# ai4co/rl4co

Hardware: NVIDIA H100
Metric: node-selections/sec TSP-100 AM rollout (higher is better)
Workload: dtype f32

## Files before the change

### include/corollout.h

```cpp
#ifndef COROLLOUT_H_
#define COROLLOUT_H_

#include <stdint.h>

#ifdef __cplusplus
extern "C" {
#endif

#define CO_VERSION 100

#define CO_OK 0
#define CO_ERR_BAD_ARG (-1)
#define CO_ERR_UNSUPPORTED (-2)
#define CO_ERR_CUDA (-3)

#define CO_EMBED_DIM 128
#define CO_NUM_HEADS 8

#define CO_ENV_TSP 0
#define CO_ENV_CVRP 1
#define CO_ENV_SDVRP 2
#define CO_ENV_OP 3
#define CO_ENV_PCTSP 4

#define CO_SELECT_GREEDY 0
#define CO_SELECT_SAMPLE_NOISE 1
#define CO_SELECT_EVALUATE 2
#define CO_SELECT_SAMPLE_PHILOX 3

int co_version(void);
const char* co_last_error_string(void);
int co_device_sm_count(void);


int co_tsp_step(const int64_t* action, const uint8_t* mask_in, uint8_t* mask_out,
                int64_t* first_node, int64_t* current_node, int64_t* i, uint8_t* done,
                int B, int N, void* stream);

int co_cvrp_action_mask(const float* demand, const float* used_capacity,
                        const float* vehicle_capacity, const uint8_t* visited,
                        const int64_t* current_node, uint8_t* mask_out, int B, int N,
                        void* stream);

int co_cvrp_step(const int64_t* action, const float* demand, const float* vehicle_capacity,
                 const float* used_in, float* used_out, const uint8_t* visited_in,
                 uint8_t* visited_out, int64_t* current_node, uint8_t* done,
                 uint8_t* mask_out, int B, int N, void* stream);

int co_sdvrp_action_mask(const float* demand_with_depot, const float* used_capacity,
                         const float* vehicle_capacity, const int64_t* current_node, uint8_t* mask_out,
                         int B, int N, void* stream);
int co_sdvrp_step(const int64_t* action, const float* demand_in, float* demand_out,
                  const float* vehicle_capacity, const float* used_in, float* used_out,
                  int64_t* current_node, uint8_t* done, uint8_t* mask_out, int B, int N, void* stream);

int co_op_action_mask(const float* locs, const float* max_length, const uint8_t* visited, const float* tour_length,
                      const int64_t* current_node, uint8_t* mask_out, int B, int N, void* stream);
int co_op_step(const int64_t* action, const float* locs, const float* prize, const float* max_length,
               const uint8_t* visited_in, uint8_t* visited_out, float* tour_length, float* current_total_prize,
               int64_t* current_node, int64_t* i, uint8_t* done, uint8_t* mask_out, int B, int N, void* stream);
int co_op_reward(const float* prize, const int64_t* actions, float* reward, int B, int N, int T, void* stream);

int co_pctsp_action_mask(const uint8_t* visited, const float* cur_total_prize, uint8_t* mask_out, int B, int N, void* stream);
int co_pctsp_step(const int64_t* action, const float* real_prize, const float* penalty, const uint8_t* visited_in,
                  uint8_t* visited_out, float* cur_total_prize, float* cur_total_penalty, int64_t* current_node, int64_t* i,
                  uint8_t* done, uint8_t* mask_out, int B, int N, void* stream);

int co_tour_length(const float* locs, const int64_t* actions, float* reward, int B,
                   int B_locs, int N, int T, int with_depot, void* stream);

int co_check_tours(const int64_t* actions, const float* demand,
                   const float* vehicle_capacity, int32_t* bad_count, int B, int B_inst,
                   int N, int T, void* stream);

#define CO_TWO_OPT_MAX_NODES 1024
#define CO_TWO_OPT_RESIDENT_MAX_NODES 224
int co_tsp_two_opt(const float* locs, const float* dist, const int64_t* tours_in, int64_t* tours_out,
                   int32_t* iterations, int B, int N, int max_iterations, void* stream);

int co_cvrp_local_search(const float* locs, const float* dist, const float* demand, const float* capacity,
                         const int64_t* tours_in, int64_t* tours_out, int32_t* used_len, int32_t* iterations,
                         int32_t* feasible, int B, int N, int T, int max_iterations, void* stream);


typedef struct co_decoder_weights {
  const float* project_context_t;
  const float* w_placeholder;
  const float* project_out_t;
  const float* dynamic_w;
  const float* dynamic_feature;
} co_decoder_weights;

int co_pointer_logits(int env_kind, const co_decoder_weights* w, const float* node_emb,
                      const float* graph_ctx ,
                      const float* glimpse_key, const float* glimpse_val,
                      const float* logit_key, const uint8_t* action_mask,
                      const int64_t* first_node, const int64_t* current_node,
                      const int64_t* i, const float* used_capacity,
                      const float* vehicle_capacity, float* logits_out, int B_traj,
                      int B_inst, int N, int ld, void* stream);

int co_select_action(const float* logits, const uint8_t* action_mask, const float* noise,
                     int64_t* action_io, float* logp_out, float* logprobs_out, int mode,
                     float tanh_clipping, float temperature, int mask_logits,
                     uint64_t seed, uint64_t offset, int B, int N, void* stream);


#define CO_ROLLOUT_FORCED_START 1
#define CO_ROLLOUT_NO_PREFETCH 2

typedef struct co_rollout_args {
  int32_t env_kind;
  int32_t select_mode;
  int32_t B_inst;
  int32_t num_starts;
  int32_t N;
  int32_t T_max;
  int32_t num_loc;
  int32_t flags;
  float tanh_clipping;
  float temperature;
  const float* cache;
  const float* graph_ctx;
  const float* q_placeholder;
  const float* w_capacity;
  const float* locs;
  const float* demand;
  const float* vehicle_capacity;
  const int64_t* forced_actions;
  const float* noise;
  uint64_t seed, offset;
  int64_t* actions_out;
  float* logp_out;
  float* reward_out;
  float* loglik_out;
  int32_t* steps_out;
  int32_t* max_steps_out;
  float* used_capacity_out;
  const float* node_emb;
  const float* w_first;
  int32_t cache_width;
  int32_t reserved0;
  const float* dyn_w;
  const float* node_limit;
} co_rollout_args;

typedef struct co_eas_grad_args {
  int32_t env_kind;
  int32_t B_inst;
  int32_t num_rows;
  int32_t N;
  int32_t T;
  int32_t cache_width;
  float tanh_clipping;
  float temperature;
  const float* cache;
  const float* graph_ctx;
  const float* w_capacity;
  const float* demand;
  const float* vehicle_capacity;
  const int64_t* actions;
  const float* coef;
  float* dLf;
  float* loglik;
  int32_t* bad_rows;
} co_eas_grad_args;
int co_eas_key_grad(const co_eas_grad_args* args, void* stream);

int co_cache_width(int env_kind);
int co_rollout_max_nodes(void);
int co_rollout(const co_rollout_args* args, void* stream);

int co_split_tf32(const float* w, float* hi, float* lo, long n, void* stream);
int co_gemm_tf32x3(const float* A, const float* Whi, const float* Wlo, float* C,
                   const float* bias, const float* residual, const float* scale,
                   const float* shift, int M, int Nout, int K, int lda, int ldc, int ldr,
                   int relu, void* stream);

long co_ffn_tiled_weight_floats(void);
int co_ffn_tile_weights(const float* w1hi, const float* w1lo, const float* w2hi, const float* w2lo, float* wtiled,
                        void* stream);
int co_ffn_fused(const float* x, const float* wtiled, const float* b1, const float* b2, const float* scale,
                 const float* shift, float* out, int M, int ldx, int ldo, void* stream);

int co_generate_uniform(float* out, long n, uint64_t seed, uint64_t offset, float lo, float hi, void* stream);
int co_generate_demand(float* out, long n, uint64_t seed, uint64_t offset, int min_demand, int max_demand,
                       float capacity, void* stream);
int co_dihedral8(const float* locs, float* out, long B, int N, void* stream);

int co_symmetric_augment(const float* base, const float* phi, float* out, long B, int S, int N, void* stream);

#define CO_LOCS_MAX_NODES 10000
#define CO_LOCS_UNIFORM 0
#define CO_LOCS_CONSTANT 1
#define CO_LOCS_NORMAL 2
#define CO_LOCS_CLUSTER 3
#define CO_LOCS_MIXED 4
#define CO_LOCS_GAUSSIAN_MIXTURE 5
#define CO_LOCS_MIX_DISTRIBUTION 6
#define CO_LOCS_MIX_MULTI_DISTRIBUTIONS 7
typedef struct co_locs_args {
  int64_t B;
  int32_t N;
  int32_t kind;
  uint64_t seed, offset;
  float lo, hi;
  float mean, std;
  int32_t n_cluster;
  int32_t n_cluster_mix;
  int32_t num_modes;
  float cdist;
} co_locs_args;
int co_generate_locs(float* out, const co_locs_args* args, void* stream);

int co_encoder_mha(const float* qkv, float* out, int B, int N, void* stream);

typedef struct co_attn_args {
  const float* q;
  const float* k;
  const float* v;
  const uint32_t* mask;
  float* o;
  float* lse;
  const float* dO;
  float* dq;
  float* dk;
  float* dv;
  int32_t B, M, N, reserved0;
  int64_t q_bs, k_bs, v_bs, o_bs, dq_bs, dk_bs, dv_bs;
  int32_t q_rs, k_rs, v_rs, o_rs, dq_rs, dk_rs, dv_rs;
  float scale;
} co_attn_args;
int co_attn_fwd(const co_attn_args* args, void* stream);
int co_attn_bwd(const co_attn_args* args, void* stream);

int co_instance_norm(const float* x, const float* gamma, const float* beta, float* out, long B, int N, float eps,
                     void* stream);

int co_reward_stats(const float* reward, double* out2, int B, void* stream);

#ifdef __cplusplus
}
#endif
#endif
```

### rl4co_b200/csrc/gemm_tf32x3.cu

```cuda
#include "co_common.cuh"
#include "wgmma.cuh"

namespace co {

constexpr int GM = 128, GN = 128, GK = 32;
constexpr int TILE_BYTES = GM * GK * 4;
constexpr uint32_t SBO = 1024;
constexpr int KB128 = 4;
constexpr int STAGES = 3;
constexpr int GEMM_THREADS = 384;
constexpr int GEMM_SMEM = 2 * KB128 * TILE_BYTES + STAGES * 2 * TILE_BYTES;

__device__ __forceinline__ float4 split_hi(float4 v) {
  return make_float4(wg::rna_tf32(v.x), wg::rna_tf32(v.y), wg::rna_tf32(v.z), wg::rna_tf32(v.w));
}
__device__ __forceinline__ float4 sub4(float4 a, float4 b) { return make_float4(a.x - b.x, a.y - b.y, a.z - b.z, a.w - b.w); }

__global__ void split_tf32_kernel(const float* __restrict__ w, float* __restrict__ hi, float* __restrict__ lo, long n) {
  long i = (long)blockIdx.x * blockDim.x + threadIdx.x;
  if (i < n) {
    const float v = w[i], h = wg::rna_tf32(v);
    hi[i] = h;
    lo[i] = v - h;
  }
}

struct GemmArgs {
  const float* A; const float* Whi; const float* Wlo; float* C;
  const float* bias; const float* residual; const float* scale; const float* shift;
  int M, Nout, K, lda, ldc, ldr, relu, n_tiles;
};

__device__ __forceinline__ void epilogue_regs(const GemmArgs& g, const float (&d)[64], int m0, int n0, int lane) {
  const int q = lane & 3;
#pragma unroll
  for (int j = 0; j < 16; ++j) {
    const int n = n0 + 8 * j + 2 * q;
    if (n >= g.Nout) continue;
    float2 bs = make_float2(0.f, 0.f), sc = make_float2(1.f, 1.f), sh = bs;
    if (g.bias) bs = __ldg(reinterpret_cast<const float2*>(g.bias + n));
    if (g.scale) { sc = __ldg(reinterpret_cast<const float2*>(g.scale + n)); sh = __ldg(reinterpret_cast<const float2*>(g.shift + n)); }
#pragma unroll
    for (int half = 0; half < 2; ++half) {
      const int row = m0 + (lane >> 2) + 8 * half;
      if (row >= g.M) continue;
      float2 o = make_float2(d[4 * j + 2 * half] + bs.x, d[4 * j + 2 * half + 1] + bs.y);
      if (g.residual) {
        const float2 r = *reinterpret_cast<const float2*>(g.residual + (size_t)row * g.ldr + n);
        o.x += r.x; o.y += r.y;
      }
      if (g.relu) { o.x = fmaxf(o.x, 0.f); o.y = fmaxf(o.y, 0.f); }
      if (g.scale) { o.x = fmaf(o.x, sc.x, sh.x); o.y = fmaf(o.y, sc.y, sh.y); }
      *reinterpret_cast<float2*>(g.C + (size_t)row * g.ldc + n) = o;
    }
  }
}

template <bool WSTAT>
struct KBlock {
  float4 a[8];
  float4 h[WSTAT ? 1 : 8], l[WSTAT ? 1 : 8];
};

template <bool WSTAT>
__global__ void __launch_bounds__(GEMM_THREADS, 1) gemm_tf32x3_kernel(const GemmArgs g, int m_tiles, int groups) {
  extern __shared__ __align__(1024) unsigned char smem[];
  constexpr int STAGE_BYTES = (WSTAT ? 2 : 4) * TILE_BYTES;
  unsigned char* sW = smem;
  unsigned char* sRing = smem + (WSTAT ? 2 * KB128 * TILE_BYTES : 0);
  __shared__ __align__(8) uint64_t bars[2 * STAGES];

  const int tid = threadIdx.x, warp = tid >> 5, lane = tid & 31;
  const int n_tile = blockIdx.x % g.n_tiles, group = blockIdx.x / g.n_tiles;
  const int n0 = n_tile * GN;
  const int nkb = g.K / GK;
  const uint32_t bar0 = wg::s32(bars);
  auto FULL_B = [&](int s) { return bar0 + 8 * s; };
  auto EMPTY_B = [&](int s) { return bar0 + 8 * (STAGES + s); };

  if (tid == 0) {
    for (int s = 0; s < STAGES; ++s) { wg::bar_init(FULL_B(s), 128); wg::bar_init(EMPTY_B(s), 256); }
    wg::bar_init_fence();
  }
  if (WSTAT) {
    const int r8 = lane & 7, c4 = lane >> 3;
    for (int item = warp; item < KB128 * 32; item += GEMM_THREADS / 32) {
      const int kb = item >> 5, qq = item & 31;
      const int rg = qq >> 1, chunk = 4 * (qq & 1) + c4, row = 8 * rg + r8;
      const uint32_t soff = rg * SBO + r8 * 128 + ((chunk ^ r8) << 4);
      float4 h = make_float4(0.f, 0.f, 0.f, 0.f), l = h;
      if (n0 + row < g.Nout) {
        h = __ldg(reinterpret_cast<const float4*>(g.Whi + (size_t)(n0 + row) * g.K + kb * GK + chunk * 4));
        l = __ldg(reinterpret_cast<const float4*>(g.Wlo + (size_t)(n0 + row) * g.K + kb * GK + chunk * 4));
      }
      *reinterpret_cast<float4*>(sW + (2 * kb) * TILE_BYTES + soff) = h;
      *reinterpret_cast<float4*>(sW + (2 * kb + 1) * TILE_BYTES + soff) = l;
    }
    wg::fence_async();
  }
  __syncthreads();

  if (warp < 4) {
    const int r4 = lane >> 3, c8 = lane & 7;
    auto load = [&](int mt, int kb, auto& R) {
#pragma unroll
      for (int j = 0; j < 8; ++j) {
        const int lrow = 16 * j + 4 * warp + r4;
        const int row = mt * GM + lrow;
        R.a[j] = make_float4(0.f, 0.f, 0.f, 0.f);
        if (mt < m_tiles && row < g.M)
          R.a[j] = __ldg(reinterpret_cast<const float4*>(g.A + (size_t)row * g.lda + kb * GK + c8 * 4));
        if constexpr (!WSTAT) {
          R.h[j] = R.l[j] = make_float4(0.f, 0.f, 0.f, 0.f);
          if (mt < m_tiles && n0 + lrow < g.Nout) {
            R.h[j] = __ldg(reinterpret_cast<const float4*>(g.Whi + (size_t)(n0 + lrow) * g.K + kb * GK + c8 * 4));
            R.l[j] = __ldg(reinterpret_cast<const float4*>(g.Wlo + (size_t)(n0 + lrow) * g.K + kb * GK + c8 * 4));
          }
        }
      }
    };
    KBlock<WSTAT> R;
    KBlock<true> Rn;
    load(group, 0, R);
    uint32_t it = 0;
    for (int mt = group; mt < m_tiles; mt += groups) {
      for (int kb = 0; kb < nkb; ++kb, ++it) {
        auto load_next = [&](auto& dst) { if (kb + 1 < nkb) load(mt, kb + 1, dst); else load(mt + groups, 0, dst); };
        if constexpr (WSTAT) load_next(Rn);
        const int s = it % STAGES;
        wg::bar_wait(EMPTY_B(s), ((it / STAGES) & 1) ^ 1);
        unsigned char* st = sRing + s * STAGE_BYTES;
#pragma unroll
        for (int j = 0; j < 8; ++j) {
          const int lrow = 16 * j + 4 * warp + r4;
          const uint32_t soff = (lrow >> 3) * SBO + (lrow & 7) * 128 + ((c8 ^ (lrow & 7)) << 4);
          const float4 h = split_hi(R.a[j]);
          *reinterpret_cast<float4*>(st + soff) = h;
          *reinterpret_cast<float4*>(st + TILE_BYTES + soff) = sub4(R.a[j], h);
          if (!WSTAT) {
            *reinterpret_cast<float4*>(st + 2 * TILE_BYTES + soff) = R.h[j];
            *reinterpret_cast<float4*>(st + 3 * TILE_BYTES + soff) = R.l[j];
          }
        }
        wg::fence_async();
        wg::bar_arrive(FULL_B(s));
        if constexpr (WSTAT) R = Rn; else load_next(R);
      }
    }
  } else {
    const int cw = (warp - 4) >> 2, w4 = warp & 3;
    uint32_t it = 0;
    float d[64];
    for (int mt = group; mt < m_tiles; mt += groups) {
      for (int kb = 0; kb < nkb; ++kb, ++it) {
        const int s = it % STAGES;
        wg::bar_wait(FULL_B(s), (it / STAGES) & 1);
        const uint32_t ahi = wg::s32(sRing + s * STAGE_BYTES) + cw * 64 * 128, alo = ahi + TILE_BYTES;
        const uint32_t bhi = WSTAT ? wg::s32(sW + (2 * kb) * TILE_BYTES) : wg::s32(sRing + s * STAGE_BYTES + 2 * TILE_BYTES);
        const uint32_t blo = bhi + TILE_BYTES;
        wg::pin(d);
        wg::fence();
#pragma unroll
        for (int kk = 0; kk < GK / 8; ++kk) {
          const uint32_t off = kk * 32;
          wg::mma_ss_n128(d, wg::desc_sw128(ahi + off, SBO), wg::desc_sw128(bhi + off, SBO), (kb | kk) != 0);
          wg::mma_ss_n128(d, wg::desc_sw128(alo + off, SBO), wg::desc_sw128(bhi + off, SBO), 1);
          wg::mma_ss_n128(d, wg::desc_sw128(ahi + off, SBO), wg::desc_sw128(blo + off, SBO), 1);
        }
        wg::commit();
        if (kb > 0) {
          wg::wait<1>();
          wg::bar_arrive(EMPTY_B((it - 1) % STAGES));
        }
      }
      wg::wait<0>();
      wg::pin(d);
      wg::bar_arrive(EMPTY_B((it - 1) % STAGES));
      epilogue_regs(g, d, mt * GM + 64 * cw + 16 * w4, n0, lane);
    }
  }
}

}

using namespace co;

extern "C" int co_split_tf32(const float* w, float* hi, float* lo, long n, void* stream) {
  if (!w || !hi || !lo || n < 0) return fail(CO_ERR_BAD_ARG, "co_split_tf32: bad argument%s");
  if (n == 0) return CO_OK;
  split_tf32_kernel<<<(unsigned)((n + 255) / 256), 256, 0, (cudaStream_t)stream>>>(w, hi, lo, n);
  return check_launch("co_split_tf32");
}

extern "C" int co_gemm_tf32x3(const float* A, const float* Whi, const float* Wlo, float* C, const float* bias,
                              const float* residual, const float* scale, const float* shift, int M, int Nout, int K,
                              int lda, int ldc, int ldr, int relu, void* stream) {
  if (!A || !Whi || !Wlo || !C) return fail(CO_ERR_BAD_ARG, "co_gemm_tf32x3: null pointer%s");
  if (M < 0 || Nout <= 0 || K <= 0) return fail(CO_ERR_BAD_ARG, "co_gemm_tf32x3: bad shape%s");
  if ((K % GK) || (Nout % 4) || (lda % 4) || (ldc % 4) || (residual && (ldr % 4)))
    return fail(CO_ERR_UNSUPPORTED, "co_gemm_tf32x3: K %% 32, Nout %% 4 and 16-byte row strides required%s");
  if ((scale == nullptr) != (shift == nullptr)) return fail(CO_ERR_BAD_ARG, "co_gemm_tf32x3: scale and shift go together%s");
  if (((uintptr_t)A | (uintptr_t)Whi | (uintptr_t)Wlo | (uintptr_t)C | (uintptr_t)bias | (uintptr_t)residual |
       (uintptr_t)scale | (uintptr_t)shift) & 15)
    return fail(CO_ERR_BAD_ARG, "co_gemm_tf32x3: pointers must be 16-byte aligned%s");
  if (M == 0) return CO_OK;
  GemmArgs g{A, Whi, Wlo, C, bias, residual, scale, shift, M, Nout, K, lda, ldc, ldr, relu, (Nout + GN - 1) / GN};
  const int m_tiles = (M + GM - 1) / GM;
  if ((long)m_tiles * g.n_tiles > 0x7fffffffL) return fail(CO_ERR_UNSUPPORTED, "co_gemm_tf32x3: too many tiles%s");
  static PerDeviceOnce once;
  bool& configured = once.flag();
  if (!configured) {
    cudaError_t e = cudaFuncSetAttribute(gemm_tf32x3_kernel<true>, cudaFuncAttributeMaxDynamicSharedMemorySize, GEMM_SMEM);
    if (e == cudaSuccess)
      e = cudaFuncSetAttribute(gemm_tf32x3_kernel<false>, cudaFuncAttributeMaxDynamicSharedMemorySize, STAGES * 4 * TILE_BYTES);
    if (e != cudaSuccess) return fail(CO_ERR_CUDA, "co_gemm_tf32x3: smem attribute: %s", cudaGetErrorString(e));
    configured = true;
  }
  int groups = device_info().sm_count / g.n_tiles;
  if (groups < 1) groups = 1;
  if (groups > m_tiles) groups = m_tiles;
  if (K == GK * KB128)
    gemm_tf32x3_kernel<true><<<groups * g.n_tiles, GEMM_THREADS, GEMM_SMEM, (cudaStream_t)stream>>>(g, m_tiles, groups);
  else
    gemm_tf32x3_kernel<false><<<groups * g.n_tiles, GEMM_THREADS, STAGES * 4 * TILE_BYTES, (cudaStream_t)stream>>>(g, m_tiles, groups);
  return check_launch("co_gemm_tf32x3");
}
```

### rl4co_b200/native.py

```python

from __future__ import annotations

import ctypes
import os
import subprocess
import sys
from ctypes import POINTER, Structure, c_char_p, c_float, c_int, c_int32, c_uint64, c_void_p

import torch

_HERE = os.path.dirname(os.path.abspath(__file__))
CSRC = os.path.join(_HERE, "csrc")
INCLUDE = os.path.join(os.path.dirname(_HERE), "include")
LIB_PATH = os.path.join(_HERE, "libcorollout.so")
SOURCES = ["abi.cu", "env_kernels.cu", "decode_step.cu", "rollout.cu", "rollout_tsp.cu", "rollout_cvrp.cu", "rollout_ms_tsp.cu", "rollout_ms_cvrp.cu", "rollout_sdvrp.cu", "rollout_op.cu", "rollout_pctsp.cu", "gemm_tf32x3.cu",
           "encoder_mha.cu", "encoder_mha_wgmma.cu",
           "ffn_fused.cu", "data_kernels.cu", "attn_train.cu", "norm_kernels.cu", "op_kernels.cu", "local_search.cu", "eas_kernels.cu"]
HEADERS = ["co_common.cuh", "rollout_impl.cuh", "rollout_ms_impl.cuh", "wgmma.cuh"]

CO_OK = 0
ENV_TSP, ENV_CVRP = 0, 1
ENV_SDVRP = 2
ENV_OP, ENV_PCTSP = 3, 4
ENV_KIND = {"tsp": ENV_TSP, "cvrp": ENV_CVRP, "sdvrp": ENV_SDVRP, "op": ENV_OP, "pctsp": ENV_PCTSP}
ROLLOUT_ENVS = ("tsp", "cvrp", "sdvrp", "op", "pctsp")
SELECT_GREEDY, SELECT_SAMPLE_NOISE, SELECT_EVALUATE, SELECT_SAMPLE_PHILOX = 0, 1, 2, 3
ROLLOUT_FORCED_START = 1
EMBED_DIM, NUM_HEADS = 128, 8

EXPORTS = [
    "co_version", "co_last_error_string", "co_device_sm_count", "co_tsp_step", "co_cvrp_action_mask",
    "co_cvrp_step", "co_tour_length", "co_check_tours", "co_pointer_logits", "co_select_action",
    "co_cache_width", "co_rollout_max_nodes", "co_rollout", "co_reward_stats", "co_split_tf32", "co_gemm_tf32x3", "co_encoder_mha",
    "co_ffn_fused", "co_ffn_tile_weights", "co_ffn_tiled_weight_floats", "co_generate_uniform", "co_generate_demand", "co_dihedral8",
    "co_sdvrp_step", "co_sdvrp_action_mask", "co_attn_fwd", "co_attn_bwd", "co_instance_norm", "co_op_step", "co_op_action_mask", "co_op_reward", "co_pctsp_step", "co_pctsp_action_mask",
    "co_tsp_two_opt", "co_generate_locs", "co_symmetric_augment", "co_cvrp_local_search",
    "co_eas_key_grad",
]


class NativeLibraryError(RuntimeError):
    pass


class DecoderWeights(Structure):
    _fields_ = [("project_context_t", c_void_p), ("w_placeholder", c_void_p), ("project_out_t", c_void_p),
                ("dynamic_w", c_void_p), ("dynamic_feature", c_void_p)]


class RolloutArgs(Structure):
    _fields_ = [
        ("env_kind", c_int32), ("select_mode", c_int32), ("B_inst", c_int32), ("num_starts", c_int32),
        ("N", c_int32), ("T_max", c_int32), ("num_loc", c_int32), ("flags", c_int32),
        ("tanh_clipping", c_float), ("temperature", c_float),
        ("cache", c_void_p), ("graph_ctx", c_void_p), ("q_placeholder", c_void_p), ("w_capacity", c_void_p),
        ("locs", c_void_p), ("demand", c_void_p), ("vehicle_capacity", c_void_p),
        ("forced_actions", c_void_p), ("noise", c_void_p), ("seed", c_uint64), ("offset", c_uint64),
        ("actions_out", c_void_p), ("logp_out", c_void_p), ("reward_out", c_void_p), ("loglik_out", c_void_p),
        ("steps_out", c_void_p), ("max_steps_out", c_void_p), ("used_capacity_out", c_void_p),
        ("node_emb", c_void_p), ("w_first", c_void_p), ("cache_width", c_int32), ("reserved0", c_int32),
        ("dyn_w", c_void_p), ("node_limit", c_void_p),
    ]


class EasGradArgs(Structure):
    _fields_ = [("env_kind", c_int32), ("B_inst", c_int32), ("num_rows", c_int32), ("N", c_int32), ("T", c_int32),
                ("cache_width", c_int32), ("tanh_clipping", c_float), ("temperature", c_float)] + [
        (n, c_void_p) for n in ("cache", "graph_ctx", "w_capacity", "demand", "vehicle_capacity", "actions", "coef",
                                "dLf", "loglik", "bad_rows")]


class AttnArgs(Structure):
    _fields_ = ([(n, c_void_p) for n in ("q", "k", "v", "mask", "o", "lse", "dO", "dq", "dk", "dv")]
                + [(n, c_int32) for n in ("B", "M", "N", "reserved0")]
                + [(n, ctypes.c_int64) for n in ("q_bs", "k_bs", "v_bs", "o_bs", "dq_bs", "dk_bs", "dv_bs")]
                + [(n, c_int32) for n in ("q_rs", "k_rs", "v_rs", "o_rs", "dq_rs", "dk_rs", "dv_rs")]
                + [("scale", c_float)])


class LocsArgs(Structure):
    _fields_ = [("B", ctypes.c_int64), ("N", c_int32), ("kind", c_int32), ("seed", c_uint64), ("offset", c_uint64),
                ("lo", c_float), ("hi", c_float), ("mean", c_float), ("std", c_float), ("n_cluster", c_int32),
                ("n_cluster_mix", c_int32), ("num_modes", c_int32), ("cdist", c_float)]


LOCS_KIND = {"uniform": 0, "constant": 1, "normal": 2, "cluster": 3, "mixed": 4, "gaussian_mixture": 5,
             "mix_distribution": 6, "mix_multi_distributions": 7}
LOCS_MAX_NODES = 10000


NVCC_FLAGS = ["-gencode", "arch=compute_90a,code=sm_90a", "-O3", "-lineinfo", "-std=c++17",
              "-Xcompiler", "-fPIC", "-I", INCLUDE]


def _nvcc() -> str:
    nvcc = os.environ.get("NVCC", "/usr/local/cuda/bin/nvcc")
    return nvcc if os.path.exists(nvcc) else "nvcc"


def build(force: bool = False, verbose: bool = False, extra_flags: list[str] | None = None) -> str:
    deps = [os.path.join(CSRC, s) for s in SOURCES + HEADERS] + [os.path.join(INCLUDE, "corollout.h")]
    if not force and os.path.exists(LIB_PATH) and all(os.path.getmtime(LIB_PATH) >= os.path.getmtime(s) for s in deps):
        return LIB_PATH
    objdir = os.path.join(_HERE, "build")
    os.makedirs(objdir, exist_ok=True)
    procs = []
    for s in SOURCES:
        obj = os.path.join(objdir, s.replace(".cu", ".o"))
        cmd = [_nvcc()] + NVCC_FLAGS + (extra_flags or []) + ["-c", os.path.join(CSRC, s), "-o", obj]
        if verbose:
            print(" ".join(cmd), file=sys.stderr)
        procs.append((s, obj, subprocess.Popen(cmd, stdout=subprocess.PIPE, stderr=subprocess.STDOUT, text=True)))
    objs, log = [], []
    for s, obj, p in procs:
        out, _ = p.communicate()
        log.append(out)
        if p.returncode != 0:
            raise NativeLibraryError(f"nvcc failed on {s} ({p.returncode}):\n{out}")
        objs.append(obj)
    link = [_nvcc(), "-gencode", "arch=compute_90a,code=sm_90a", "-shared", "-o", LIB_PATH] + objs
    res = subprocess.run(link, capture_output=True, text=True)
    if res.returncode != 0:
        raise NativeLibraryError(f"link failed ({res.returncode}):\n{res.stdout}\n{res.stderr}")
    build.last_log = "\n".join(log)
    return LIB_PATH


_lib = None


def lib() -> ctypes.CDLL:
    global _lib
    if _lib is not None:
        return _lib
    if not os.path.exists(LIB_PATH):
        raise NativeLibraryError(
            f"{LIB_PATH} not found: run `python -c 'import __graft_entry__ as g; g.build()'` "
            "(there is no CPU/PyTorch fallback for the rollout path)")
    L = ctypes.CDLL(LIB_PATH)
    for name in EXPORTS:
        if not hasattr(L, name):
            raise NativeLibraryError(f"{LIB_PATH} does not export {name}")
    L.co_last_error_string.restype = c_char_p
    L.co_rollout.argtypes = [POINTER(RolloutArgs), c_void_p]
    L.co_pointer_logits.argtypes = [c_int, POINTER(DecoderWeights)] + [c_void_p] * 12 + [c_int, c_int, c_int, c_int, c_void_p]
    L.co_select_action.argtypes = [c_void_p] * 6 + [c_int, c_float, c_float, c_int, c_uint64, c_uint64, c_int, c_int, c_void_p]
    L.co_tsp_step.argtypes = [c_void_p] * 7 + [c_int, c_int, c_void_p]
    L.co_cvrp_action_mask.argtypes = [c_void_p] * 6 + [c_int, c_int, c_void_p]
    L.co_cvrp_step.argtypes = [c_void_p] * 10 + [c_int, c_int, c_void_p]
    L.co_tour_length.argtypes = [c_void_p] * 3 + [c_int] * 5 + [c_void_p]
    L.co_sdvrp_action_mask.argtypes = [c_void_p] * 5 + [c_int, c_int, c_void_p]
    L.co_sdvrp_step.argtypes = [c_void_p] * 9 + [c_int, c_int, c_void_p]
    L.co_check_tours.argtypes = [c_void_p] * 4 + [c_int] * 4 + [c_void_p]
    L.co_tsp_two_opt.argtypes = [c_void_p] * 5 + [c_int] * 3 + [c_void_p]
    L.co_cvrp_local_search.argtypes = [c_void_p] * 9 + [c_int] * 4 + [c_void_p]
    L.co_reward_stats.argtypes = [c_void_p, c_void_p, c_int, c_void_p]
    L.co_op_action_mask.argtypes = [c_void_p] * 6 + [c_int, c_int, c_void_p]
    L.co_op_step.argtypes = [c_void_p] * 12 + [c_int, c_int, c_void_p]
    L.co_pctsp_action_mask.argtypes = [c_void_p] * 3 + [c_int, c_int, c_void_p]
    L.co_pctsp_step.argtypes = [c_void_p] * 11 + [c_int, c_int, c_void_p]
    L.co_op_reward.argtypes = [c_void_p] * 3 + [c_int, c_int, c_int, c_void_p]
    L.co_instance_norm.argtypes = [c_void_p, c_void_p, c_void_p, c_void_p, ctypes.c_long, c_int, c_float, c_void_p]
    L.co_eas_key_grad.argtypes = [POINTER(EasGradArgs), c_void_p]
    L.co_attn_fwd.argtypes = [POINTER(AttnArgs), c_void_p]
    L.co_attn_bwd.argtypes = [POINTER(AttnArgs), c_void_p]
    L.co_cache_width.argtypes = [c_int]
    L.co_split_tf32.argtypes = [c_void_p, c_void_p, c_void_p, ctypes.c_long, c_void_p]
    L.co_gemm_tf32x3.argtypes = [c_void_p] * 8 + [c_int] * 7 + [c_void_p]
    L.co_encoder_mha.argtypes = [c_void_p, c_void_p, c_int, c_int, c_void_p]
    L.co_ffn_fused.argtypes = [c_void_p] * 7 + [c_int, c_int, c_int, c_void_p]
    L.co_ffn_tile_weights.argtypes = [c_void_p] * 5 + [c_void_p]
    L.co_ffn_tiled_weight_floats.restype = ctypes.c_long
    L.co_generate_uniform.argtypes = [c_void_p, ctypes.c_long, c_uint64, c_uint64, c_float, c_float, c_void_p]
    L.co_generate_demand.argtypes = [c_void_p, ctypes.c_long, c_uint64, c_uint64, c_int, c_int, c_float, c_void_p]
    L.co_dihedral8.argtypes = [c_void_p, c_void_p, ctypes.c_long, c_int, c_void_p]
    L.co_symmetric_augment.argtypes = [c_void_p, c_void_p, c_void_p, ctypes.c_long, c_int, c_int, c_void_p]
    L.co_generate_locs.argtypes = [c_void_p, POINTER(LocsArgs), c_void_p]
    _lib = L
    return L


LAUNCH_COUNT = 0


def _check(rc: int, what: str) -> None:
    global LAUNCH_COUNT
    LAUNCH_COUNT += 1
    if rc != CO_OK:
        msg = lib().co_last_error_string().decode("utf-8", "replace")
        raise NativeLibraryError(f"{what} failed with code {rc}: {msg}")


def _ptr(t: torch.Tensor | None, dtype: torch.dtype | None = None, name: str = "tensor", strided: bool = False):
    if t is None:
        return None
    if not isinstance(t, torch.Tensor):
        raise TypeError(f"{name}: expected a torch.Tensor, got {type(t)}")
    if not t.is_cuda:
        raise NativeLibraryError(f"{name}: libcorollout needs CUDA tensors (got device {t.device}); "
                                 "there is no CPU fallback")
    if dtype is not None and t.dtype != dtype:
        raise TypeError(f"{name}: expected dtype {dtype}, got {t.dtype}")
    if not strided and not t.is_contiguous():
        raise ValueError(f"{name}: tensor must be contiguous")
    return t.data_ptr()


def _stream():
    return torch.cuda.current_stream().cuda_stream


def _on_device_of_first_tensor(fn):
    import functools

    @functools.wraps(fn)
    def wrapper(*args, **kwargs):
        for a in list(args) + list(kwargs.values()):
            if isinstance(a, torch.Tensor) and a.is_cuda:
                if a.device.index != torch.cuda.current_device():
                    with torch.cuda.device(a.device):
                        return fn(*args, **kwargs)
                break
        return fn(*args, **kwargs)

    return wrapper


F32, I64, U8, I32 = torch.float32, torch.int64, torch.uint8, torch.int32


def _bool_ptr(t, name):
    if t is None:
        return None
    if t.dtype not in (torch.bool, torch.uint8):
        raise TypeError(f"{name}: expected bool/uint8, got {t.dtype}")
    return _ptr(t, None, name)




def version() -> int:
    return lib().co_version()


def cache_width(env_name: str) -> int:
    return lib().co_cache_width(ENV_KIND[env_name])


def rollout_max_nodes() -> int:
    return lib().co_rollout_max_nodes()


@_on_device_of_first_tensor
def tsp_step(action, mask_in, mask_out, first_node, current_node, i, done):
    B, N = mask_in.shape
    _check(lib().co_tsp_step(_ptr(action, I64, "action"), _bool_ptr(mask_in, "mask_in"), _bool_ptr(mask_out, "mask_out"),
                             _ptr(first_node, I64, "first_node"), _ptr(current_node, I64, "current_node"),
                             _ptr(i, I64, "i"), _bool_ptr(done, "done"), B, N, _stream()), "co_tsp_step")


@_on_device_of_first_tensor
def cvrp_action_mask(demand, used, cap, visited, current_node, mask_out):
    B, N = visited.shape
    _check(lib().co_cvrp_action_mask(_ptr(demand, F32, "demand"), _ptr(used, F32, "used"), _ptr(cap, F32, "cap"),
                                     _ptr(visited, U8, "visited"), _ptr(current_node, I64, "current_node"),
                                     _bool_ptr(mask_out, "mask_out"), B, N, _stream()), "co_cvrp_action_mask")


@_on_device_of_first_tensor
def cvrp_step(action, demand, cap, used_in, used_out, visited_in, visited_out, current_node, done, mask_out):
    B, N = visited_in.shape
    _check(lib().co_cvrp_step(_ptr(action, I64, "action"), _ptr(demand, F32, "demand"), _ptr(cap, F32, "cap"),
                              _ptr(used_in, F32, "used_in"), _ptr(used_out, F32, "used_out"),
                              _ptr(visited_in, U8, "visited_in"), _ptr(visited_out, U8, "visited_out"),
                              _ptr(current_node, I64, "current_node"), _bool_ptr(done, "done"),
                              _bool_ptr(mask_out, "mask_out"), B, N, _stream()), "co_cvrp_step")


@_on_device_of_first_tensor
def sdvrp_action_mask(demand_with_depot, used, cap, current_node, mask_out):
    B, N = demand_with_depot.shape
    _check(lib().co_sdvrp_action_mask(_ptr(demand_with_depot, F32, "demand_with_depot"), _ptr(used, F32, "used_capacity"),
                                      _ptr(cap, F32, "vehicle_capacity"), _ptr(current_node, I64, "current_node"),
                                      _bool_ptr(mask_out, "mask_out"), B, N, _stream()), "co_sdvrp_action_mask")
    return mask_out


@_on_device_of_first_tensor
def sdvrp_step(action, demand_in, demand_out, cap, used_in, used_out, current_node, done, mask_out):
    B, N = demand_in.shape
    _check(lib().co_sdvrp_step(_ptr(action, I64, "action"), _ptr(demand_in, F32, "demand_in"),
                               _ptr(demand_out, F32, "demand_out"), _ptr(cap, F32, "vehicle_capacity"),
                               _ptr(used_in, F32, "used_in"), _ptr(used_out, F32, "used_out"),
                               _ptr(current_node, I64, "current_node"), _bool_ptr(done, "done"),
                               _bool_ptr(mask_out, "mask_out"), B, N, _stream()), "co_sdvrp_step")


@_on_device_of_first_tensor
def op_action_mask(locs, max_length, visited, tour_length, current_node, mask_out):
    B, N = mask_out.shape
    _check(lib().co_op_action_mask(_ptr(locs, F32, "locs"), _ptr(max_length, F32, "max_length"), _bool_ptr(visited, "visited"),
                                   _ptr(tour_length, F32, "tour_length"), _ptr(current_node, I64, "current_node"),
                                   _bool_ptr(mask_out, "mask_out"), B, N, _stream()), "co_op_action_mask")
    return mask_out


@_on_device_of_first_tensor
def op_step(action, locs, prize, max_length, visited_in, visited_out, tour_length, current_total_prize, current_node, i,
            done, mask_out):
    B, N = mask_out.shape
    _check(lib().co_op_step(_ptr(action, I64, "action"), _ptr(locs, F32, "locs"), _ptr(prize, F32, "prize"),
                            _ptr(max_length, F32, "max_length"), _bool_ptr(visited_in, "visited_in"),
                            _bool_ptr(visited_out, "visited_out"), _ptr(tour_length, F32, "tour_length"),
                            _ptr(current_total_prize, F32, "current_total_prize"), _ptr(current_node, I64, "current_node"),
                            _ptr(i, I64, "i"), _bool_ptr(done, "done"), _bool_ptr(mask_out, "mask_out"), B, N, _stream()),
           "co_op_step")


@_on_device_of_first_tensor
def pctsp_action_mask(visited, cur_total_prize, mask_out):
    B, N = mask_out.shape
    _check(lib().co_pctsp_action_mask(_bool_ptr(visited, "visited"), _ptr(cur_total_prize, F32, "cur_total_prize"),
                                      _bool_ptr(mask_out, "mask_out"), B, N, _stream()), "co_pctsp_action_mask")
    return mask_out


@_on_device_of_first_tensor
def pctsp_step(action, real_prize, penalty, visited_in, visited_out, cur_total_prize, cur_total_penalty, current_node, i, done,
               mask_out):
    B, N = mask_out.shape
    _check(lib().co_pctsp_step(_ptr(action, I64, "action"), _ptr(real_prize, F32, "real_prize"), _ptr(penalty, F32, "penalty"),
                               _bool_ptr(visited_in, "visited_in"), _bool_ptr(visited_out, "visited_out"),
                               _ptr(cur_total_prize, F32, "cur_total_prize"), _ptr(cur_total_penalty, F32, "cur_total_penalty"),
                               _ptr(current_node, I64, "current_node"), _ptr(i, I64, "i"), _bool_ptr(done, "done"),
                               _bool_ptr(mask_out, "mask_out"), B, N, _stream()), "co_pctsp_step")


@_on_device_of_first_tensor
def op_reward(prize, actions):
    B, T = actions.shape
    if prize.shape[0] != B:
        prize = prize.repeat(B // prize.shape[0], 1)
    out = torch.empty(B, dtype=F32, device=actions.device)
    _check(lib().co_op_reward(_ptr(prize.contiguous(), F32, "prize"), _ptr(actions, I64, "actions"), _ptr(out, F32, "reward"),
                              B, prize.shape[1], T, _stream()), "co_op_reward")
    return out


@_on_device_of_first_tensor
def tour_length(locs, actions, with_depot: bool):
    B, T = actions.shape
    B_locs, N = locs.shape[0], locs.shape[1]
    reward = torch.empty(B, dtype=F32, device=actions.device)
    _check(lib().co_tour_length(_ptr(locs, F32, "locs"), _ptr(actions, I64, "actions"), _ptr(reward, F32, "reward"),
                                B, B_locs, N, T, int(with_depot), _stream()), "co_tour_length")
    return reward


@_on_device_of_first_tensor
def check_tours(actions, N, demand=None, cap=None, B_inst=None) -> int:
    B, T = actions.shape
    bad = torch.zeros(1, dtype=I32, device=actions.device)
    _check(lib().co_check_tours(_ptr(actions, I64, "actions"), _ptr(demand, F32, "demand"), _ptr(cap, F32, "cap"),
                                _ptr(bad, I32, "bad"), B, B if B_inst is None else B_inst, N, T, _stream()),
           "co_check_tours")
    return int(bad.item())


@_on_device_of_first_tensor
def tsp_two_opt(tours, max_iterations: int = 1000, locs=None, distances=None, iterations=None):
    if (locs is None) == (distances is None):
        raise ValueError("tsp_two_opt: pass exactly one of locs / distances")
    if tours.dim() != 2:
        raise ValueError(f"tours: expected [B, N], got {tuple(tours.shape)}")
    B, N = tours.shape
    if locs is not None and tuple(locs.shape) != (B, N, 2):
        raise ValueError(f"locs: expected [{B}, {N}, 2], got {tuple(locs.shape)}")
    if distances is not None and tuple(distances.shape) != (B, N, N):
        raise ValueError(f"distances: expected [{B}, {N}, {N}], got {tuple(distances.shape)}")
    if iterations is not None and tuple(iterations.shape) != (B,):
        raise ValueError(f"iterations: expected [{B}], got {tuple(iterations.shape)}")
    out = torch.empty(B, N, dtype=I64, device=tours.device)
    _check(lib().co_tsp_two_opt(_ptr(locs, F32, "locs"), _ptr(distances, F32, "distances"), _ptr(tours, I64, "tours"),
                                _ptr(out, I64, "tours_out"), _ptr(iterations, I32, "iterations"), B, N,
                                min(int(max_iterations), 2**31 - 1), _stream()), "co_tsp_two_opt")
    return out


@_on_device_of_first_tensor
def cvrp_local_search(tours, demand, capacity, max_iterations: int, locs=None, distances=None, iterations=None,
                      feasible=None):
    if (locs is None) == (distances is None):
        raise ValueError("cvrp_local_search: pass exactly one of locs / distances")
    if tours.dim() != 2:
        raise ValueError(f"tours: expected [B, T], got {tuple(tours.shape)}")
    B, T = tours.shape
    if demand.dim() != 2 or demand.shape[0] != B:
        raise ValueError(f"demand: expected [{B}, N], got {tuple(demand.shape)}")
    N = demand.shape[1]
    if tuple(capacity.shape) != (B,):
        raise ValueError(f"capacity: expected [{B}], got {tuple(capacity.shape)}")
    if locs is not None and tuple(locs.shape) != (B, N + 1, 2):
        raise ValueError(f"locs: expected [{B}, {N + 1}, 2], got {tuple(locs.shape)}")
    if distances is not None and tuple(distances.shape) != (B, N + 1, N + 1):
        raise ValueError(f"distances: expected [{B}, {N + 1}, {N + 1}], got {tuple(distances.shape)}")
    for name, t in (("iterations", iterations), ("feasible", feasible)):
        if t is not None and tuple(t.shape) != (B,):
            raise ValueError(f"{name}: expected [{B}], got {tuple(t.shape)}")
    out = torch.empty(B, 2 * N, dtype=I64, device=tours.device)
    used = torch.empty(B, dtype=I32, device=tours.device)
    _check(lib().co_cvrp_local_search(_ptr(locs, F32, "locs"), _ptr(distances, F32, "distances"),
                                      _ptr(demand, F32, "demand"), _ptr(capacity, F32, "capacity"),
                                      _ptr(tours, I64, "tours"), _ptr(out, I64, "tours_out"), _ptr(used, I32, "used"),
                                      _ptr(iterations, I32, "iterations"), _ptr(feasible, I32, "feasible"), B, N, T,
                                      min(int(max_iterations), 2**31 - 1), _stream()), "co_cvrp_local_search")
    return out, used


@_on_device_of_first_tensor
def eas_key_grad(env_name, cache, actions, coef, graph_ctx=None, w_capacity=None, demand=None, vehicle_capacity=None,
                 tanh_clipping=10.0, temperature=1.0, bad_rows=None):
    if env_name not in ("tsp", "cvrp"):
        raise NotImplementedError(f"co_eas_key_grad covers tsp and cvrp, not {env_name!r}")
    if cache.dim() != 3:
        raise ValueError(f"cache: expected [B_inst, N, W], got {tuple(cache.shape)}")
    B_inst, N, W = cache.shape
    if actions.dim() != 2 or B_inst == 0 or actions.shape[0] % max(B_inst, 1) or actions.shape[0] == 0:
        raise ValueError(f"actions: expected [R * {B_inst}, T], got {tuple(actions.shape)}")
    R, T = actions.shape[0] // B_inst, actions.shape[1]
    if tuple(coef.shape) != (R * B_inst,):
        raise ValueError(f"coef: expected [{R * B_inst}], got {tuple(coef.shape)}")
    if graph_ctx is not None and tuple(graph_ctx.shape) != (B_inst, EMBED_DIM):
        raise ValueError(f"graph_ctx: expected [{B_inst}, {EMBED_DIM}], got {tuple(graph_ctx.shape)}")
    if env_name == "cvrp":
        if w_capacity is None or demand is None:
            raise ValueError("cvrp needs w_capacity and demand")
        if tuple(w_capacity.shape) != (EMBED_DIM,) or tuple(demand.shape) != (B_inst, N - 1):
            raise ValueError(f"w_capacity must be [{EMBED_DIM}] and demand [{B_inst}, {N - 1}]")
        if vehicle_capacity is not None and tuple(vehicle_capacity.shape) != (B_inst,):
            raise ValueError(f"vehicle_capacity: expected [{B_inst}], got {tuple(vehicle_capacity.shape)}")
    if bad_rows is not None and tuple(bad_rows.shape) != (1,):
        raise ValueError("bad_rows: expected an int32 [1] counter")
    dLf = torch.empty(B_inst, N, EMBED_DIM, dtype=F32, device=cache.device)
    loglik = torch.empty(R * B_inst, dtype=F32, device=cache.device)
    a = EasGradArgs()
    a.env_kind, a.B_inst, a.num_rows, a.N, a.T, a.cache_width = ENV_KIND[env_name], B_inst, R, N, T, W
    a.tanh_clipping, a.temperature = float(tanh_clipping), float(temperature)
    a.cache = _ptr(cache, F32, "cache")
    a.graph_ctx = _ptr(graph_ctx, F32, "graph_ctx")
    a.w_capacity = _ptr(w_capacity, F32, "w_capacity") if env_name == "cvrp" else None
    a.demand = _ptr(demand, F32, "demand") if env_name == "cvrp" else None
    a.vehicle_capacity = _ptr(vehicle_capacity, F32, "vehicle_capacity") if env_name == "cvrp" else None
    a.actions = _ptr(actions, I64, "actions")
    a.coef = _ptr(coef, F32, "coef")
    a.dLf, a.loglik = _ptr(dLf, F32, "dLf"), _ptr(loglik, F32, "loglik")
    a.bad_rows = _ptr(bad_rows, I32, "bad_rows")
    _check(lib().co_eas_key_grad(ctypes.byref(a), _stream()), "co_eas_key_grad")
    return dLf, loglik


@_on_device_of_first_tensor
def pointer_logits(env_name, weights: DecoderWeights, node_emb, graph_ctx, K, V, L, mask, first_node, current_node,
                   i, used, cap, B_traj, B_inst, N):
    ld = K.stride(1)
    for name, x in (("glimpse_key", K), ("glimpse_val", V), ("logit_key", L)):
        if x.stride(2) != 1 or x.stride(1) != ld or x.stride(0) != N * ld:
            raise ValueError(f"{name}: unsupported strides {x.stride()}")
    logits = torch.empty(B_traj, N, dtype=F32, device=node_emb.device)
    _check(lib().co_pointer_logits(ENV_KIND["cvrp" if env_name in ("op", "pctsp") else env_name], ctypes.byref(weights), _ptr(node_emb, F32, "node_emb"),
                                   _ptr(graph_ctx, F32, "graph_ctx"), _ptr(K, F32, "glimpse_key", True),
                                   _ptr(V, F32, "glimpse_val", True), _ptr(L, F32, "logit_key", True),
# ... 267 lines not shown
```

Measured before the change: 103.7 million.

## Add ping-pong consumer warpgroups to the W-stationary TF32x3 GEMM

For K=128, the GEMM now runs two consumer warpgroups on alternating M-tiles, handing off through named barriers so one group's epilogue overlaps the other's MMAs. Registers are rebalanced with setmaxnreg, the next A tile is prefetched into L2, and the epilogue uses quad-shuffled float4 stores. The old cooperative path stays available as a separate entry point. This adds barrier-ordering complexity and register-pressure risk in exchange for hiding epilogue latency in the encoder GEMMs.

Result: faster. 105.8 million, median of 6 (+2.0%).

```diff
diff --git a/include/corollout.h b/include/corollout.h
--- a/include/corollout.h
+++ b/include/corollout.h
@@ -176,6 +176,10 @@
                    const float* bias, const float* residual, const float* scale,
                    const float* shift, int M, int Nout, int K, int lda, int ldc, int ldr,
                    int relu, void* stream);
+int co_gemm_tf32x3_coop(const float* A, const float* Whi, const float* Wlo, float* C,
+                        const float* bias, const float* residual, const float* scale,
+                        const float* shift, int M, int Nout, int K, int lda, int ldc, int ldr,
+                        int relu, void* stream);
 
 long co_ffn_tiled_weight_floats(void);
 int co_ffn_tile_weights(const float* w1hi, const float* w1lo, const float* w2hi, const float* w2lo, float* wtiled,
diff --git a/rl4co_b200/csrc/gemm_tf32x3.cu b/rl4co_b200/csrc/gemm_tf32x3.cu
--- a/rl4co_b200/csrc/gemm_tf32x3.cu
+++ b/rl4co_b200/csrc/gemm_tf32x3.cu
@@ -56,14 +56,45 @@
   }
 }
 
+__device__ __forceinline__ void epilogue_quad(const GemmArgs& g, const float (&d)[64], int m0, int n0, int lane) {
+  const int q = lane & 3, odd = q & 1;
+  const int row = m0 + (lane >> 2) + 8 * odd;
+#pragma unroll
+  for (int j = 0; j < 16; ++j) {
+    const float sx = odd ? d[4 * j] : d[4 * j + 2], sy = odd ? d[4 * j + 1] : d[4 * j + 3];
+    const float rx = __shfl_xor_sync(0xffffffffu, sx, 1), ry = __shfl_xor_sync(0xffffffffu, sy, 1);
+    const int n = n0 + 8 * j + 2 * (q & 2);
+    if (n >= g.Nout || row >= g.M) continue;
+    float4 v = odd ? make_float4(rx, ry, d[4 * j + 2], d[4 * j + 3]) : make_float4(d[4 * j], d[4 * j + 1], rx, ry);
+    if (g.bias) {
+      const float4 bs = __ldg(reinterpret_cast<const float4*>(g.bias + n));
+      v.x += bs.x; v.y += bs.y; v.z += bs.z; v.w += bs.w;
+    } else {
+      v.x += 0.f; v.y += 0.f; v.z += 0.f; v.w += 0.f;
+    }
+    if (g.residual) {
+      const float4 r = *reinterpret_cast<const float4*>(g.residual + (size_t)row * g.ldr + n);
+      v.x += r.x; v.y += r.y; v.z += r.z; v.w += r.w;
+    }
+    if (g.relu) { v.x = fmaxf(v.x, 0.f); v.y = fmaxf(v.y, 0.f); v.z = fmaxf(v.z, 0.f); v.w = fmaxf(v.w, 0.f); }
+    if (g.scale) {
+      const float4 sc = __ldg(reinterpret_cast<const float4*>(g.scale + n)), sh = __ldg(reinterpret_cast<const float4*>(g.shift + n));
+      v.x = fmaf(v.x, sc.x, sh.x); v.y = fmaf(v.y, sc.y, sh.y); v.z = fmaf(v.z, sc.z, sh.z); v.w = fmaf(v.w, sc.w, sh.w);
+    }
+    *reinterpret_cast<float4*>(g.C + (size_t)row * g.ldc + n) = v;
+  }
+}
+
 template <bool WSTAT>
 struct KBlock {
   float4 a[8];
   float4 h[WSTAT ? 1 : 8], l[WSTAT ? 1 : 8];
 };
 
-template <bool WSTAT>
+template <bool WSTAT, bool PP>
 __global__ void __launch_bounds__(GEMM_THREADS, 1) gemm_tf32x3_kernel(const GemmArgs g, int m_tiles, int groups) {
+  static_assert(WSTAT || !PP, "ping-pong needs the W-stationary ring");
+  static_assert(!PP || KB128 > STAGES, "ping-pong ordering: a tile spans more k-blocks than the ring has stages");
   extern __shared__ __align__(1024) unsigned char smem[];
   constexpr int STAGE_BYTES = (WSTAT ? 2 : 4) * TILE_BYTES;
   unsigned char* sW = smem;
@@ -79,7 +110,7 @@
   auto EMPTY_B = [&](int s) { return bar0 + 8 * (STAGES + s); };
 
   if (tid == 0) {
-    for (int s = 0; s < STAGES; ++s) { wg::bar_init(FULL_B(s), 128); wg::bar_init(EMPTY_B(s), 256); }
+    for (int s = 0; s < STAGES; ++s) { wg::bar_init(FULL_B(s), 128); wg::bar_init(EMPTY_B(s), PP ? 128 : 256); }
     wg::bar_init_fence();
   }
   if (WSTAT) {
@@ -101,20 +132,32 @@
   __syncthreads();
 
   if (warp < 4) {
+    if constexpr (PP) asm volatile("setmaxnreg.dec.sync.aligned.u32 128;\n" ::: "memory");
     const int r4 = lane >> 3, c8 = lane & 7;
     auto load = [&](int mt, int kb, auto& R) {
-#pragma unroll
-      for (int j = 0; j < 8; ++j) {
-        const int lrow = 16 * j + 4 * warp + r4;
-        const int row = mt * GM + lrow;
-        R.a[j] = make_float4(0.f, 0.f, 0.f, 0.f);
-        if (mt < m_tiles && row < g.M)
-          R.a[j] = __ldg(reinterpret_cast<const float4*>(g.A + (size_t)row * g.lda + kb * GK + c8 * 4));
-        if constexpr (!WSTAT) {
-          R.h[j] = R.l[j] = make_float4(0.f, 0.f, 0.f, 0.f);
-          if (mt < m_tiles && n0 + lrow < g.Nout) {
-            R.h[j] = __ldg(reinterpret_cast<const float4*>(g.Whi + (size_t)(n0 + lrow) * g.K + kb * GK + c8 * 4));
-            R.l[j] = __ldg(reinterpret_cast<const float4*>(g.Wlo + (size_t)(n0 + lrow) * g.K + kb * GK + c8 * 4));
+      if constexpr (PP) {
+        const int row0 = mt * GM + 4 * warp + r4;
+        const int rows = mt < m_tiles ? g.M - row0 : 0;
+        const float* p = g.A + (size_t)row0 * g.lda + kb * GK + c8 * 4;
+#pragma unroll
+        for (int j = 0; j < 8; ++j) {
+          R.a[j] = make_float4(0.f, 0.f, 0.f, 0.f);
+          if (16 * j < rows) R.a[j] = __ldg(reinterpret_cast<const float4*>(p + (size_t)(16 * j) * g.lda));
+        }
+      } else {
+#pragma unroll
+        for (int j = 0; j < 8; ++j) {
+          const int lrow = 16 * j + 4 * warp + r4;
+          const int row = mt * GM + lrow;
+          R.a[j] = make_float4(0.f, 0.f, 0.f, 0.f);
+          if (mt < m_tiles && row < g.M)
+            R.a[j] = __ldg(reinterpret_cast<const float4*>(g.A + (size_t)row * g.lda + kb * GK + c8 * 4));
+          if constexpr (!WSTAT) {
+            R.h[j] = R.l[j] = make_float4(0.f, 0.f, 0.f, 0.f);
+            if (mt < m_tiles && n0 + lrow < g.Nout) {
+              R.h[j] = __ldg(reinterpret_cast<const float4*>(g.Whi + (size_t)(n0 + lrow) * g.K + kb * GK + c8 * 4));
+              R.l[j] = __ldg(reinterpret_cast<const float4*>(g.Wlo + (size_t)(n0 + lrow) * g.K + kb * GK + c8 * 4));
+            }
           }
         }
       }
@@ -124,6 +167,12 @@
     load(group, 0, R);
     uint32_t it = 0;
     for (int mt = group; mt < m_tiles; mt += groups) {
+      if constexpr (PP) {
+        const int prow = (mt + groups) * GM + tid;
+        if (g.n_tiles > 1 && mt + groups < m_tiles && prow < g.M)
+          asm volatile("cp.async.bulk.prefetch.L2.global [%0], %1;" ::"l"(g.A + (size_t)prow * g.lda), "r"(GK * KB128 * 4)
+                       : "memory");
+      }
       for (int kb = 0; kb < nkb; ++kb, ++it) {
         auto load_next = [&](auto& dst) { if (kb + 1 < nkb) load(mt, kb + 1, dst); else load(mt + groups, 0, dst); };
         if constexpr (WSTAT) load_next(Rn);
@@ -146,6 +195,47 @@
         wg::bar_arrive(FULL_B(s));
         if constexpr (WSTAT) R = Rn; else load_next(R);
       }
+    }
+  } else if constexpr (PP) {
+    asm volatile("setmaxnreg.inc.sync.aligned.u32 184;\n" ::: "memory");
+    const int cw = (warp - 4) >> 2, w4 = warp & 3;
+    float d0[64], d1[64];
+    for (int lt = cw, mt = group + cw * groups; mt < m_tiles; lt += 2, mt += 2 * groups) {
+      if (lt > 0) asm volatile("bar.sync %0, 256;" ::"r"(1 + cw) : "memory");
+      uint32_t it = lt * nkb;
+      for (int kb = 0; kb < nkb; ++kb, ++it) {
+        const int s = it % STAGES;
+        wg::bar_wait(FULL_B(s), (it / STAGES) & 1);
+        const uint32_t ahi = wg::s32(sRing + s * STAGE_BYTES), alo = ahi + TILE_BYTES;
+        const uint32_t bhi = wg::s32(sW + (2 * kb) * TILE_BYTES), blo = bhi + TILE_BYTES;
+        wg::pin(d0);
+        wg::pin(d1);
+        wg::fence();
+#pragma unroll
+        for (int kk = 0; kk < GK / 8; ++kk) {
+          const uint32_t off = kk * 32, h64 = 64 * 128;
+          const uint64_t bh = wg::desc_sw128(bhi + off, SBO), bl = wg::desc_sw128(blo + off, SBO);
+          wg::mma_ss_n128(d0, wg::desc_sw128(ahi + off, SBO), bh, (kb | kk) != 0);
+          wg::mma_ss_n128(d1, wg::desc_sw128(ahi + h64 + off, SBO), bh, (kb | kk) != 0);
+          wg::mma_ss_n128(d0, wg::desc_sw128(alo + off, SBO), bh, 1);
+          wg::mma_ss_n128(d1, wg::desc_sw128(alo + h64 + off, SBO), bh, 1);
+          wg::mma_ss_n128(d0, wg::desc_sw128(ahi + off, SBO), bl, 1);
+          wg::mma_ss_n128(d1, wg::desc_sw128(ahi + h64 + off, SBO), bl, 1);
+        }
+        wg::commit();
+        if (kb > 0) {
+          wg::wait<1>();
+          wg::bar_arrive(EMPTY_B((it - 1) % STAGES));
+        }
+      }
+      if (mt + groups < m_tiles)
+        asm volatile("bar.arrive %0, 256;" ::"r"(2 - cw) : "memory");
+      wg::wait<0>();
+      wg::pin(d0);
+      wg::pin(d1);
+      wg::bar_arrive(EMPTY_B((it - 1) % STAGES));
+      epilogue_quad(g, d0, mt * GM + 16 * w4, n0, lane);
+      epilogue_quad(g, d1, mt * GM + 64 + 16 * w4, n0, lane);
     }
   } else {
     const int cw = (warp - 4) >> 2, w4 = warp & 3;
@@ -192,36 +282,59 @@
   return check_launch("co_split_tf32");
 }
 
+namespace {
+
+int gemm_launch(const char* name, bool pp, const float* A, const float* Whi, const float* Wlo, float* C, const float* bias,
+                const float* residual, const float* scale, const float* shift, int M, int Nout, int K, int lda, int ldc,
+                int ldr, int relu, void* stream) {
+  if (!A || !Whi || !Wlo || !C) return fail(CO_ERR_BAD_ARG, "%s: null pointer", name);
+  if (M < 0 || Nout <= 0 || K <= 0) return fail(CO_ERR_BAD_ARG, "%s: bad shape", name);
+  if ((K % GK) || (Nout % 4) || (lda % 4) || (ldc % 4) || (residual && (ldr % 4)))
+    return fail(CO_ERR_UNSUPPORTED, "%s: K %% 32, Nout %% 4 and 16-byte row strides required", name);
+  if ((scale == nullptr) != (shift == nullptr)) return fail(CO_ERR_BAD_ARG, "%s: scale and shift go together", name);
+  if (((uintptr_t)A | (uintptr_t)Whi | (uintptr_t)Wlo | (uintptr_t)C | (uintptr_t)bias | (uintptr_t)residual |
+       (uintptr_t)scale | (uintptr_t)shift) & 15)
+    return fail(CO_ERR_BAD_ARG, "%s: pointers must be 16-byte aligned", name);
+  if (M == 0) return CO_OK;
+  GemmArgs g{A, Whi, Wlo, C, bias, residual, scale, shift, M, Nout, K, lda, ldc, ldr, relu, (Nout + GN - 1) / GN};
+  const int m_tiles = (M + GM - 1) / GM;
+  if ((long)m_tiles * g.n_tiles > 0x7fffffffL) return fail(CO_ERR_UNSUPPORTED, "%s: too many tiles", name);
+  static PerDeviceOnce once;
+  bool& configured = once.flag();
+  if (!configured) {
+    cudaError_t e = cudaFuncSetAttribute(gemm_tf32x3_kernel<true, true>, cudaFuncAttributeMaxDynamicSharedMemorySize, GEMM_SMEM);
+    if (e == cudaSuccess)
+      e = cudaFuncSetAttribute(gemm_tf32x3_kernel<true, false>, cudaFuncAttributeMaxDynamicSharedMemorySize, GEMM_SMEM);
+    if (e == cudaSuccess)
+      e = cudaFuncSetAttribute(gemm_tf32x3_kernel<false, false>, cudaFuncAttributeMaxDynamicSharedMemorySize, STAGES * 4 * TILE_BYTES);
+    if (e != cudaSuccess) return fail(CO_ERR_CUDA, "co_gemm_tf32x3: smem attribute: %s", cudaGetErrorString(e));
+    configured = true;
+  }
+  int groups = device_info().sm_count / g.n_tiles;
+  if (groups < 1) groups = 1;
+  if (groups > m_tiles) groups = m_tiles;
+  const cudaStream_t st = (cudaStream_t)stream;
+  if (K == GK * KB128 && pp)
+    gemm_tf32x3_kernel<true, true><<<groups * g.n_tiles, GEMM_THREADS, GEMM_SMEM, st>>>(g, m_tiles, groups);
+  else if (K == GK * KB128)
+    gemm_tf32x3_kernel<true, false><<<groups * g.n_tiles, GEMM_THREADS, GEMM_SMEM, st>>>(g, m_tiles, groups);
+  else
+    gemm_tf32x3_kernel<false, false><<<groups * g.n_tiles, GEMM_THREADS, STAGES * 4 * TILE_BYTES, st>>>(g, m_tiles, groups);
+  return check_launch(name);
+}
+
+}
+
 extern "C" int co_gemm_tf32x3(const float* A, const float* Whi, const float* Wlo, float* C, const float* bias,
                               const float* residual, const float* scale, const float* shift, int M, int Nout, int K,
                               int lda, int ldc, int ldr, int relu, void* stream) {
-  if (!A || !Whi || !Wlo || !C) return fail(CO_ERR_BAD_ARG, "co_gemm_tf32x3: null pointer%s");
-  if (M < 0 || Nout <= 0 || K <= 0) return fail(CO_ERR_BAD_ARG, "co_gemm_tf32x3: bad shape%s");
-  if ((K % GK) || (Nout % 4) || (lda % 4) || (ldc % 4) || (residual && (ldr % 4)))
-    return fail(CO_ERR_UNSUPPORTED, "co_gemm_tf32x3: K %% 32, Nout %% 4 and 16-byte row strides required%s");
-  if ((scale == nullptr) != (shift == nullptr)) return fail(CO_ERR_BAD_ARG, "co_gemm_tf32x3: scale and shift go together%s");
-  if (((uintptr_t)A | (uintptr_t)Whi | (uintptr_t)Wlo | (uintptr_t)C | (uintptr_t)bias | (uintptr_t)residual |
-       (uintptr_t)scale | (uintptr_t)shift) & 15)
-    return fail(CO_ERR_BAD_ARG, "co_gemm_tf32x3: pointers must be 16-byte aligned%s");
-  if (M == 0) return CO_OK;
-  GemmArgs g{A, Whi, Wlo, C, bias, residual, scale, shift, M, Nout, K, lda, ldc, ldr, relu, (Nout + GN - 1) / GN};
-  const int m_tiles = (M + GM - 1) / GM;
-  if ((long)m_tiles * g.n_tiles > 0x7fffffffL) return fail(CO_ERR_UNSUPPORTED, "co_gemm_tf32x3: too many tiles%s");
-  static PerDeviceOnce once;
-  bool& configured = once.flag();
-  if (!configured) {
-    cudaError_t e = cudaFuncSetAttribute(gemm_tf32x3_kernel<true>, cudaFuncAttributeMaxDynamicSharedMemorySize, GEMM_SMEM);
-    if (e == cudaSuccess)
-      e = cudaFuncSetAttribute(gemm_tf32x3_kernel<false>, cudaFuncAttributeMaxDynamicSharedMemorySize, STAGES * 4 * TILE_BYTES);
-    if (e != cudaSuccess) return fail(CO_ERR_CUDA, "co_gemm_tf32x3: smem attribute: %s", cudaGetErrorString(e));
-    configured = true;
-  }
-  int groups = device_info().sm_count / g.n_tiles;
-  if (groups < 1) groups = 1;
-  if (groups > m_tiles) groups = m_tiles;
-  if (K == GK * KB128)
-    gemm_tf32x3_kernel<true><<<groups * g.n_tiles, GEMM_THREADS, GEMM_SMEM, (cudaStream_t)stream>>>(g, m_tiles, groups);
-  else
-    gemm_tf32x3_kernel<false><<<groups * g.n_tiles, GEMM_THREADS, STAGES * 4 * TILE_BYTES, (cudaStream_t)stream>>>(g, m_tiles, groups);
-  return check_launch("co_gemm_tf32x3");
-}
+  return gemm_launch("co_gemm_tf32x3", true, A, Whi, Wlo, C, bias, residual, scale, shift, M, Nout, K, lda, ldc, ldr,
+                     relu, stream);
+}
+
+extern "C" int co_gemm_tf32x3_coop(const float* A, const float* Whi, const float* Wlo, float* C, const float* bias,
+                                   const float* residual, const float* scale, const float* shift, int M, int Nout, int K,
+                                   int lda, int ldc, int ldr, int relu, void* stream) {
+  return gemm_launch("co_gemm_tf32x3_coop", false, A, Whi, Wlo, C, bias, residual, scale, shift, M, Nout, K, lda, ldc,
+                     ldr, relu, stream);
+}
diff --git a/rl4co_b200/native.py b/rl4co_b200/native.py
--- a/rl4co_b200/native.py
+++ b/rl4co_b200/native.py
@@ -31,7 +31,7 @@
 EXPORTS = [
     "co_version", "co_last_error_string", "co_device_sm_count", "co_tsp_step", "co_cvrp_action_mask",
     "co_cvrp_step", "co_tour_length", "co_check_tours", "co_pointer_logits", "co_select_action",
-    "co_cache_width", "co_rollout_max_nodes", "co_rollout", "co_reward_stats", "co_split_tf32", "co_gemm_tf32x3", "co_encoder_mha",
+    "co_cache_width", "co_rollout_max_nodes", "co_rollout", "co_reward_stats", "co_split_tf32", "co_gemm_tf32x3", "co_gemm_tf32x3_coop", "co_encoder_mha",
     "co_ffn_fused", "co_ffn_tile_weights", "co_ffn_tiled_weight_floats", "co_generate_uniform", "co_generate_demand", "co_dihedral8",
     "co_sdvrp_step", "co_sdvrp_action_mask", "co_attn_fwd", "co_attn_bwd", "co_instance_norm", "co_op_step", "co_op_action_mask", "co_op_reward", "co_pctsp_step", "co_pctsp_action_mask",
     "co_tsp_two_opt", "co_generate_locs", "co_symmetric_augment", "co_cvrp_local_search",
@@ -167,6 +167,7 @@
     L.co_cache_width.argtypes = [c_int]
     L.co_split_tf32.argtypes = [c_void_p, c_void_p, c_void_p, ctypes.c_long, c_void_p]
     L.co_gemm_tf32x3.argtypes = [c_void_p] * 8 + [c_int] * 7 + [c_void_p]
+    L.co_gemm_tf32x3_coop.argtypes = [c_void_p] * 8 + [c_int] * 7 + [c_void_p]
     L.co_encoder_mha.argtypes = [c_void_p, c_void_p, c_int, c_int, c_void_p]
     L.co_ffn_fused.argtypes = [c_void_p] * 7 + [c_int, c_int, c_int, c_void_p]
     L.co_ffn_tile_weights.argtypes = [c_void_p] * 5 + [c_void_p]
```
